# biod/sambamba

Measured on AMD Instinct MI355X. Metric: depth_base_Mreads_per_s, higher is better.
Workload: dtype u8/u32

## Files before the change

sambamba_amd/csrc/inflate.hip:

```cpp
#include <cstdlib>

#include "common.hpp"
#include "inflate2_core.hpp"
#include "lz77_copy.hpp"
#include "kernels.hpp"

namespace sbx {

namespace {

constexpr int kInfThreads = 64;
constexpr int kLaneLds = 356;
constexpr int kLitSymOff = 0;
constexpr int kLitSymBytes = 324;
constexpr int kRingOff = 324;
constexpr int kClLenOff = 32;
constexpr int kLenTabBytes = 64, kDistTabBytes = 128;
constexpr int kLensScratch = 320;
constexpr int kScratchStride = inf2::kScratchBytes;
constexpr int kGeneralLensOff = inf2::kScratchTabs;
static_assert(kGeneralLensOff + kLensScratch <= kScratchStride, "scratch layout");

enum : uint32_t {
    INF_OK = 0,
// ... 456 lines not shown
            if (ncl_left) {
                br.refill();
                cl_len[kClOrder[cl_i++]] = (uint8_t)br.take(3);
                --ncl_left;
            }
            br.service();
        }
        if (dyn) {
            int k = 0;
            for (int l = 1; l <= 7; ++l)
                for (int s2 = 0; s2 < 19; ++s2)
                    if (cl_len[s2] == l) cl_sym[k++] = (uint8_t)s2;
            for (int s2 = 0; s2 < 19; ++s2) {
                uint32_t l = cl_len[s2];
#pragma unroll
                for (int q = 1; q < 8; ++q) ccnt[q] += (l == (uint32_t)q) ? 1u : 0u;
            }
            int32_t left = 1;
            bool ok = true;
#pragma unroll
            for (int l = 1; l <= 7; ++l) { left = (left << 1) - (int32_t)ccnt[l]; if (left < 0) ok = false; }
            if (!ok) { err = INF_BAD_CODELENS; active = false; dyn = false; }
        }
        {
            int i = 0;
            uint32_t prev = 0;
            const int total = nlit + ndist;
            bool more = dyn;
            while (__any(more)) {
                if (more) {
                    br.refill();
                    uint32_t code = 0, first = 0, index = 0, sym = 0xFFFFFFFFu;
                    int used = 0;
#pragma unroll
                    for (int l = 1; l <= 7; ++l) {
                        code |= (uint32_t)(br.buf >> (l - 1)) & 1u;
                        uint32_t c = ccnt[l];
                        if (used == 0 && code < first + c) {
                            sym = cl_sym[index + (code - first)];
                            used = l;
                        }
                        index += c;
                        first = (first + c) << 1;
                        code <<= 1;
                    }
                    if (sym >= 19) { err = INF_BAD_CODELENS; more = false; }
                    else {
                        br.drop(used);
                        if (sym < 16) {
                            lens[i++] = (uint8_t)sym;
                            prev = sym;
                        } else {
                            uint32_t rep, val;
                            if (sym == 16) { val = prev; rep = 3 + br.take(2); if (i == 0) { err = INF_BAD_CODELENS; more = false; rep = 0; } }
                            else if (sym == 17) { val = 0; rep = 3 + br.take(3); }
                            else { val = 0; rep = 11 + br.take(7); }
                            if (i + (int)rep > total) { err = INF_BAD_CODELENS; more = false; }
                            else {
                                for (uint32_t k = 0; k < rep; ++k) lens[i++] = (uint8_t)val;
                                prev = val;
                            }
                        }
                        if (i >= total) more = false;
                    }
                }
                br.service();
            }
            if (dyn && err == INF_OK && lens[256] == 0) err = INF_BAD_CODELENS;
            if (err != INF_OK) active = false;
        }
        bool sym_loop = huff && active;
        bool lit_in_14 = true, dist_in_12 = true;
        if (sym_loop) {
            if (!build_code<true, 14>(lens, nlit, lds, DS, CL, &lit_in_14)) { err = INF_BAD_CODELENS; active = false; sym_loop = false; }
            else if (!build_code<false, 12>(lens + nlit, ndist, lds, DS, CD, &dist_in_12)) { err = INF_BAD_CODELENS; active = false; sym_loop = false; }
        }
        uint32_t short_lit = __builtin_amdgcn_readfirstlane(__all(!sym_loop || lit_in_14) ? 1u : 0u);
        uint32_t short_dist = __builtin_amdgcn_readfirstlane(__all(!sym_loop || dist_in_12) ? 1u : 0u);
        asm volatile("" : "+s"(short_lit), "+s"(short_dist));

        if (__any(sym_loop)) do {
            br.service();
            em.flush();
            uint32_t msym = 0;
            uint32_t bad = INF_OK;
            static_assert(kLitPerIter * 15 <= 32, "one refill must cover the literal/length slots of an iteration");
            if (sym_loop) br.refill();
#pragma unroll
            for (int r = 0; r < kLitPerIter; ++r) {
                if (sym_loop && msym == 0 && bad == INF_OK) {
                    const uint32_t v = __brev((uint32_t)br.buf) >> 17;
                    int len;
                    uint32_t delta;
                    decode_len<7>(CL, v, short_lit, &len, &delta);
                    const int lc = len > 15 ? 15 : len;
                    const uint32_t idx0 = (delta + (v >> (15 - lc))) & 0x1FFu;
                    const uint32_t idx = idx0 > 287u ? 287u : idx0;
                    const uint32_t bo = 9u * idx;
                    uint16_t packed;
                    __builtin_memcpy(&packed, lds + kLitSymOff + (bo >> 3), 2);
                    const uint32_t sym = ((uint32_t)packed >> (bo & 7u)) & 0x1FFu;
                    br.drop(lc);
                    const bool ok = len <= 15 && idx0 <= 287u && sym <= 285u;
                    if (ok && sym < 256u) em.literal(sym);
                    sym_loop = !(ok && sym == 256u);
                    msym = ok && sym > 256u ? sym : 0u;
                    bad = ok ? INF_OK : INF_BAD_SYMBOL;
                }
            }
            em.park_lits();
            const uint32_t opos_now = opos + em.n_lit;
            if (opos_now > osize && bad == INF_OK) { bad = INF_OUTPUT_OVERRUN; msym = 0; }
            if (msym != 0) {
                br.refill();
                const uint32_t lt = len_tab[msym - 257u];
                const uint32_t le = lt >> 9, lb = lt & 0x1FFu;
                const uint32_t mlen = lb + br.take((int)le);
                const uint32_t dv = __brev((uint32_t)br.buf) >> 17;
                int dl;
                uint32_t ddelta;
                decode_len<6>(CD, dv, short_dist, &dl, &ddelta);
                const int dc = dl > 15 ? 15 : dl;
                const uint32_t didx0 = (ddelta + (dv >> (15 - dc))) & 0x1FFu;
                const uint32_t dsym = DS.get(didx0 > 29u ? 29u : didx0);
                br.drop(dc);
                const uint32_t dt = dist_tab[dsym];
                const uint32_t de = dt >> 16, db = dt & 0xFFFFu;
                const uint32_t dist = db + br.take((int)de);
                const bool code_ok = dl <= 15 && didx0 < 30u && dsym <= 29u && dist <= opos_now;
                const bool fits = opos_now + mlen <= osize;
                if (code_ok && fits) { opos += mlen; em.match(mlen, dist); }
                bad = !code_ok ? (uint32_t)INF_BAD_DISTANCE : !fits ? (uint32_t)INF_OUTPUT_OVERRUN : bad;
            }
            if (bad != INF_OK) { err = bad; active = false; sym_loop = false; }
        } while (__any(sym_loop));
        if (active && last) active = false;
    }
    em.finish();
    if (err == INF_OK && opos + em.n_lit != osize) err = INF_SIZE_MISMATCH;
    if (err == INF_OK && br.consumed() > in_bits) err = INF_INPUT_OVERRUN;
    if (live) {
        status[b] = err;
        n_entries[b] = em.n_ent;
    }
    if (tok_bytes) {
        unsigned long long t = live ? (unsigned long long)em.n_lit + 4ull * em.n_ent : 0ull;
        for (int d = 32; d >= 1; d >>= 1) t += __shfl_xor(t, d, 64);
        if (threadIdx.x == 0) atomicAdd(tok_bytes + (blockIdx.x & 63u), t);
    }
}


constexpr int kInf2Threads = 64;
__global__ __launch_bounds__(kInf2Threads) __attribute__((amdgpu_waves_per_eu(4, 4))) void k_huffman_decode2(
    const uint8_t* __restrict__ comp, const uint64_t* __restrict__ comp_off, const uint32_t* __restrict__ comp_len,
    const uint32_t* __restrict__ isize, const uint64_t* __restrict__ out_off, uint32_t n_blocks, uint32_t block0,
    uint8_t* __restrict__ lit_stream, uint32_t* __restrict__ ent_stream, uint32_t* __restrict__ n_entries,
    uint8_t* __restrict__ scratch, uint32_t* __restrict__ status, unsigned long long* __restrict__ tok_bytes) {
    extern __shared__ __attribute__((aligned(16))) uint8_t smem[];
    const uint32_t lane = threadIdx.x;
    const uint32_t b_raw = blockIdx.x * kInf2Threads + lane;
    const bool live = b_raw < n_blocks;
    const uint32_t b = live ? b_raw : n_blocks - 1;
    uint16_t* const len_tab = (uint16_t*)(smem + inf2::kWaveLds);
    uint32_t* const dist_tab = (uint32_t*)(smem + inf2::kWaveLds + inf2::kLenTabBytes);
    if (lane < 32u) inf2::rfc_tables_entry(lane, &len_tab[lane], &dist_tab[lane]);
    __syncthreads();
    const uint64_t oo = out_off[b];
    inf2::LaneIo io;
    io.in = comp + comp_off[b];
    io.in_bits = comp_len[b] * 8u;
    io.osize = isize[b];
    io.lit = lit_stream + lit_off(oo, block0 + b);
    io.ent = ent_stream + ent_off(oo, block0 + b);
    io.scratch = scratch + (size_t)b * kScratchStride;
    io.live = live;
    inf2::Lane L;
    const inf2::LaneResult R = L.run(io, smem, lane, len_tab, dist_tab);
    if (live) {
        status[b] = R.status;
        n_entries[b] = R.n_ent;
    }
    if (tok_bytes) {
        unsigned long long t = live && R.status == 0u ? (unsigned long long)R.n_lit + 4ull * R.n_ent : 0ull;
        for (int d = 32; d >= 1; d >>= 1) t += __shfl_xor(t, d, 64);
        if (lane == 0) atomicAdd(tok_bytes + (blockIdx.x & 63u), t);
    }
}

__global__ __launch_bounds__(64) void k_translate_literals(
    uint8_t* __restrict__ lit_stream, const uint64_t* __restrict__ out_off, uint32_t n_blocks, uint32_t block0,
    const uint8_t* __restrict__ scratch, const uint32_t* __restrict__ status) {
    __shared__ __attribute__((aligned(16))) uint8_t tabs[inf2::kMaxSeg * 256];
    __shared__ uint32_t seg_start[inf2::kMaxSeg + 1];
    const uint32_t b = blockIdx.x, lane = threadIdx.x;
    if (status[b] != INF_OK) return;
    const uint8_t* sc = scratch + (size_t)b * kScratchStride;
    const uint32_t* info = (const uint32_t*)(sc + inf2::kScratchInfo);
    const uint32_t n_seg = info[0], n_lit = info[1];
    if (n_seg == 0u || n_lit == 0u) return;
    for (uint32_t s = 0; s < n_seg; ++s) ((uint32_t*)tabs)[64u * s + lane] = ((const uint32_t*)(sc + inf2::kScratchTabs))[64u * s + lane];
    if (lane <= n_seg) seg_start[lane] = lane < n_seg ? info[2 + lane] : n_lit;
    __syncthreads();
    uint8_t* lit = lit_stream + lit_off(out_off[b], block0 + b);
    const uint32_t n_grp = (n_lit + 15u) >> 4;
    for (uint32_t g = lane; g < n_grp; g += 64) {
        u32x4 v = *(const u32x4*)(lit + 16u * g);
        const uint32_t p0 = 16u * g;
        uint32_t s0 = 0;
        while (s0 + 1u < n_seg && seg_start[s0 + 1u] <= p0) ++s0;
        const uint32_t next = seg_start[s0 + 1u];
        uint32_t w[4] = {v.x, v.y, v.z, v.w};
        if (next >= p0 + 16u || s0 + 1u >= n_seg) {
            const uint8_t* t = tabs + 256u * s0;
#pragma unroll
            for (int k = 0; k < 4; ++k) {
                const uint32_t x = w[k];
                w[k] = (uint32_t)t[x & 0xFFu] | (uint32_t)t[(x >> 8) & 0xFFu] << 8 | (uint32_t)t[(x >> 16) & 0xFFu] << 16 | (uint32_t)t[x >> 24] << 24;
            }
        } else {
            for (uint32_t i = 0; i < 16; ++i) {
                const uint32_t p = p0 + i;
                uint32_t sg = s0;
                while (sg + 1u < n_seg && seg_start[sg + 1u] <= p) ++sg;
                const uint32_t x = (w[i >> 2] >> (8u * (i & 3u))) & 0xFFu;
                const uint32_t y = tabs[256u * sg + x];
                w[i >> 2] = (w[i >> 2] & ~(0xFFu << (8u * (i & 3u)))) | y << (8u * (i & 3u));
            }
        }
        *(u32x4*)(lit + 16u * g) = u32x4{w[0], w[1], w[2], w[3]};
    }
}

constexpr int kResThreads = 256;
constexpr uint32_t kHistDefault = 2048, kSpanDefault = 1536;

__device__ __forceinline__ uint32_t wave_incl_scan(uint32_t v, uint32_t lane) {
    (void)lane;
    v += (uint32_t)__builtin_amdgcn_update_dpp(0, (int)v, 0x111, 0xF, 0xF, true);
    v += (uint32_t)__builtin_amdgcn_update_dpp(0, (int)v, 0x112, 0xF, 0xF, true);
    v += (uint32_t)__builtin_amdgcn_update_dpp(0, (int)v, 0x114, 0xF, 0xF, true);
    v += (uint32_t)__builtin_amdgcn_update_dpp(0, (int)v, 0x118, 0xF, 0xF, true);
    v += (uint32_t)__builtin_amdgcn_update_dpp(0, (int)v, 0x142, 0xA, 0xF, false);
    v += (uint32_t)__builtin_amdgcn_update_dpp(0, (int)v, 0x143, 0xC, 0xF, false);
    return v;
}

using lz::Short16;

__device__ __forceinline__ void coop_copy(uint64_t m, const uint8_t* sbase, uint32_t s, uint8_t* buf, uint32_t d, uint32_t n, uint32_t lane) {
    while (m) {
        uint32_t S[4], D[4], N[4], wa[4], wb[4];
#pragma unroll
        for (int j = 0; j < 4; ++j) {
            N[j] = 0; S[j] = 0; D[j] = 0;
            if (m) {
                const int r = __builtin_ctzll(m);
                m &= m - 1;
                S[j] = __builtin_amdgcn_readlane(s, r);
                D[j] = __builtin_amdgcn_readlane(d, r);
                N[j] = __builtin_amdgcn_readlane(n, r);
            }
        }
        const uint32_t off = 8 * lane;
#pragma unroll
        for (int j = 0; j < 4; ++j) {
            if (off < N[j]) {
                const uint32_t a = off + 4 <= N[j] ? off : N[j] - 4, c = off + 8 <= N[j] ? off + 4 : N[j] - 4;
                wa[j] = ldu32(sbase + S[j] + a);
                wb[j] = ldu32(sbase + S[j] + c);
            }
        }
#pragma unroll
        for (int j = 0; j < 4; ++j) {
            if (off < N[j]) {
                const uint32_t a = off + 4 <= N[j] ? off : N[j] - 4, c = off + 8 <= N[j] ? off + 4 : N[j] - 4;
                stu32(buf + D[j] + a, wa[j]);
                stu32(buf + D[j] + c, wb[j]);
            }
        }
    }
}

__device__ __forceinline__ void wave_copy(uint8_t* d, const uint8_t* s, uint32_t N, uint32_t lane) {
    if (N >= 4) {
        for (uint32_t off = 4 * lane; off < N; off += 256) {
            const uint32_t o2 = off + 4 <= N ? off : N - 4;
            stu32(d + o2, ldu32(s + o2));
        }
    } else if (lane < N) {
        d[lane] = s[lane];
    }
}

template <uint32_t kHist, uint32_t kSpanMax, bool kOwn32, bool kExact, uint32_t kAblate = 0, bool kTail16 = true>
__device__ __forceinline__ void lz77_resolve_body(
    const uint8_t* __restrict__ lit_stream, const uint32_t* __restrict__ ent_stream, const uint32_t* __restrict__ n_entries,
    const uint64_t* __restrict__ out_off, const uint32_t* __restrict__ isize, uint32_t n_blocks, uint32_t block0,
    uint8_t* out, const uint32_t* __restrict__ status) {
    extern __shared__ __attribute__((aligned(16))) uint8_t smem[];
    const uint32_t lane = threadIdx.x & 63u, wv = threadIdx.x >> 6;
    const uint32_t b = blockIdx.x * (kResThreads / 64) + wv;
    if (kOwn32) {
        uint32_t* tab = (uint32_t*)(smem + (kResThreads / 64) * (kHist + 1024u + kSpanMax + 16u));
        if (threadIdx.x < 32u) {
            const uint32_t d = (threadIdx.x >> 2) + 1u, j = threadIdx.x & 3u;
            tab[threadIdx.x] = lz::period_selector(d, j);
        }
        __syncthreads();
    }
    if (b >= n_blocks) return;
    if (status[b] != INF_OK) return;
    constexpr uint32_t kCap = kHist + 1024u + kSpanMax, kWaveLds = kCap + 16u;
    uint8_t* buf = smem + wv * kWaveLds;
    const uint32_t* per_sel = (const uint32_t*)(smem + (kResThreads / 64) * kWaveLds);
    const uint64_t oo = out_off[b];
    const uint8_t* lit = lit_stream + lit_off(oo, block0 + b);
    const uint32_t* ent = ent_stream + ent_off(oo, block0 + b);
    uint8_t* o = out + oo;
    const uint32_t ne = n_entries[b];
    uint32_t opos = 0, lpos = 0;
    uint32_t base = 0;

    uint32_t e_next = lane < ne ? ent[lane] : 0u;
    for (uint32_t e0 = 0; e0 < ne;) {
        uint32_t e = e_next;
        const uint32_t in_batch = ne - e0 < 64u ? ne - e0 : 64u;
        uint32_t lr = e >> 24, len = e & 511u;
        const uint32_t dist = ((e >> 9) & 0x7FFFu) + 1u;
        uint32_t tot = lr + len;
        const uint32_t pk = wave_incl_scan(tot | (lr << 16), lane);
        const uint32_t take = __popcll(__ballot(lane < in_batch && (pk & 0xFFFFu) <= kSpanMax));
        if (lane >= take) { lr = 0; len = 0; tot = 0; }
        const uint32_t pk_last = __builtin_amdgcn_readlane(pk, take - 1);
        const uint32_t span = pk_last & 0xFFFFu, lspan = pk_last >> 16;
        e0 += take;
        e_next = (e0 + lane < ne) ? ent[e0 + lane] : 0u;
        if (!(kAblate & 32u) && opos - base + kSpanMax > kCap) {
            const uint32_t nb = (opos - kHist) & ~15u, delta = nb - base, keep = opos - nb;
            for (uint32_t i = 16 * lane; i < keep; i += 1024) {
// ... 238 lines not shown
```

sambamba_amd/csrc/inflate2_core.hpp:

```cpp
#pragma once
#include <cstdint>
#include <cstring>

#if defined(__HIPCC__)
#include <hip/hip_runtime.h>
#define SBX_HD __host__ __device__ __forceinline__
#else
#define SBX_HD inline
#endif

namespace sbx {
namespace inf2 {

constexpr uint32_t kNeedsGeneral = 100;
constexpr int kMaxSeg = 6;
constexpr int kScratchLens = 0;
constexpr int kScratchInfo = 160;
constexpr int kScratchTabs = 256;
constexpr int kScratchBytes = kScratchTabs + kMaxSeg * 256;

constexpr int kRingDw = 9;
constexpr int kOffRing = 0;
constexpr int kOffLitStage = kOffRing + 256 * kRingDw;
constexpr int kOffEntStage = kOffLitStage + 256 * 4;
constexpr int kOffAux = kOffEntStage + 256 * 8;
constexpr int kSymEntries = 30;
constexpr int kOffLenSym = kOffAux + 128 * 16;
constexpr int kOffDistSym = kOffLenSym + 64 * kSymEntries;
constexpr int kWaveLds = kOffDistSym + 64 * kSymEntries;
constexpr int kLenTabBytes = 64, kDistTabBytes = 128;

constexpr uint32_t kNone = 0xFFu, kStop = 0x1FFu;

#if defined(__HIP_DEVICE_COMPILE__)
typedef short s16x2 __attribute__((ext_vector_type(2)));
typedef unsigned short u16x2 __attribute__((ext_vector_type(2)));
SBX_HD uint32_t alignbit(uint32_t hi, uint32_t lo, uint32_t s) { return __builtin_amdgcn_alignbit(hi, lo, s); }
SBX_HD uint32_t brev32(uint32_t x) { return __builtin_bitreverse32(x); }
SBX_HD bool wave_any(bool x) { return __any(x) != 0; }
SBX_HD uint32_t bfe(uint32_t x, uint32_t off, uint32_t width) { return __builtin_amdgcn_ubfe(x, off, width); }
SBX_HD uint32_t pair_mask(uint32_t lim1, uint32_t vv) {
    const s16x2 d = __builtin_bit_cast(s16x2, lim1) - __builtin_bit_cast(s16x2, vv);
    return __builtin_bit_cast(uint32_t, __builtin_bit_cast(u16x2, d) >> 15);
}
SBX_HD uint32_t pair_dot(uint32_t m, uint32_t dd, uint32_t acc) {
    return __builtin_amdgcn_udot2(__builtin_bit_cast(u16x2, m), __builtin_bit_cast(u16x2, dd), acc, false);
}
#else
SBX_HD uint32_t alignbit(uint32_t hi, uint32_t lo, uint32_t s) { return (uint32_t)(((((uint64_t)hi) << 32) | lo) >> (s & 31u)); }
SBX_HD uint32_t brev32(uint32_t x) {
    x = ((x >> 1) & 0x55555555u) | ((x & 0x55555555u) << 1);
    x = ((x >> 2) & 0x33333333u) | ((x & 0x33333333u) << 2);
    x = ((x >> 4) & 0x0F0F0F0Fu) | ((x & 0x0F0F0F0Fu) << 4);
    x = ((x >> 8) & 0x00FF00FFu) | ((x & 0x00FF00FFu) << 8);
    return (x >> 16) | (x << 16);
}
SBX_HD bool wave_any(bool x) { return x; }
SBX_HD uint32_t bfe(uint32_t x, uint32_t off, uint32_t width) { return width == 0 ? 0u : (x >> (off & 31u)) & (width >= 32 ? 0xFFFFFFFFu : ((1u << width) - 1u)); }
SBX_HD uint32_t pair_mask(uint32_t lim1, uint32_t vv) {
    const uint32_t a = (uint16_t)((uint16_t)lim1 - (uint16_t)vv), b = (uint16_t)((uint16_t)(lim1 >> 16) - (uint16_t)(vv >> 16));
    return (a >> 15) | ((b >> 15) << 16);
}
SBX_HD uint32_t pair_dot(uint32_t m, uint32_t dd, uint32_t acc) { return acc + (m & 0xFFFFu) * (dd & 0xFFFFu) + (m >> 16) * (dd >> 16); }
#endif

SBX_HD uint32_t make_entry2(uint32_t lit_run, uint32_t len, uint32_t dist) { return (lit_run << 24) | ((dist - 1u) << 9) | len; }

struct u32x4h { uint32_t x, y, z, w; };


struct Code {
    uint32_t lim1[8], dd[8];
    uint32_t d1;
    uint32_t d1_lo;
};

#if defined(__HIP_DEVICE_COMPILE__)
SBX_HD uint32_t splat16(uint32_t v) { const u16x2 x = {(unsigned short)v, (unsigned short)v}; return __builtin_bit_cast(uint32_t, x); }
#define SBX_KEEP_BRANCH() asm volatile("")
#else
SBX_HD uint32_t splat16(uint32_t v) { return v | (v << 16); }
#define SBX_KEEP_BRANCH() (void)0
#endif

template <int kFrom, int kTo>
SBX_HD uint32_t decode_pairs(const Code& C, uint32_t v, uint32_t acc) {
    const uint32_t vv = splat16(v);
    uint32_t m[kTo - kFrom > 0 ? kTo - kFrom : 1];
#pragma unroll
    for (int j = kFrom; j < kTo; ++j) m[j - kFrom] = pair_mask(C.lim1[j], vv);
#pragma unroll
    for (int j = kFrom; j < kTo; ++j) acc = pair_dot(m[j - kFrom], C.dd[j], acc);
    return acc;
}

template <bool kPlain>
SBX_HD uint32_t decode_lit(const Code& C, uint32_t v) { return kPlain ? decode_pairs<1, 7>(C, v, C.d1_lo) : decode_pairs<0, 8>(C, v, C.d1); }
template <bool kPlain>
SBX_HD uint32_t decode_dist(const Code& C, uint32_t v) { return kPlain ? decode_pairs<1, 6>(C, v, C.d1_lo) : decode_pairs<0, 8>(C, v, C.d1); }

constexpr uint64_t kClOrderLo = 16ull | 17ull << 5 | 18ull << 10 | 0ull << 15 | 8ull << 20 | 7ull << 25 | 9ull << 30 | 6ull << 35 | 10ull << 40 | 5ull << 45 | 11ull << 50 | 4ull << 55;
constexpr uint64_t kClOrderHi = 12ull | 3ull << 5 | 13ull << 10 | 2ull << 15 | 14ull << 20 | 1ull << 25 | 15ull << 30;

struct LaneIo {
    const uint8_t* in;
    uint32_t in_bits;
    uint32_t osize;
    uint8_t* lit;
    uint32_t* ent;
    uint8_t* scratch;
    bool live;
};
struct LaneResult {
    uint32_t status;
    uint32_t n_ent, n_lit;
};

struct Lane {
    uint8_t* W;
    uint32_t l4, l2, l1;
    const uint16_t* len_tab;
    const uint32_t* dist_tab;
    const uint8_t* gp;
    u32x4h pend;
    uint32_t wr_dw;
    uint32_t bitpos;
    uint32_t hi, lo;
    uint32_t n_lit, n_ent, lit_mark, opos;
    uint32_t lit_flushed, ent_flushed;
    uint8_t* lit;
    uint32_t* ent;

    SBX_HD uint32_t& dw(int off, uint32_t j) const { return *(uint32_t*)(W + off + 256u * j + l4); }
    SBX_HD uint16_t& h16(int off, uint32_t e) const { return *(uint16_t*)(W + off + 128u * e + l2); }
    SBX_HD uint8_t& b8(int off, uint32_t e) const { return W[off + 64u * e + l1]; }

    SBX_HD static u32x4h load16(const uint8_t* p) {
        u32x4h v;
#if defined(__HIP_DEVICE_COMPILE__)
        typedef uint32_t u32x4g __attribute__((ext_vector_type(4)));
        const u32x4g q = *(const __attribute__((address_space(1))) u32x4g*)(uintptr_t)p;
        v.x = q.x; v.y = q.y; v.z = q.z; v.w = q.w;
#else
        __builtin_memcpy(&v, p, 16);
#endif
        return v;
    }
    SBX_HD static void store16(void* p, u32x4h v) { __builtin_memcpy(p, &v, 16); }

    SBX_HD void put_chunk(u32x4h v) {
        const uint32_t s = wr_dw & 7u;
        dw(kOffRing, s) = v.x; dw(kOffRing, s + 1) = v.y; dw(kOffRing, s + 2) = v.z; dw(kOffRing, s + 3) = v.w;
        if (s == 0u) dw(kOffRing, 8) = v.x;
        wr_dw += 4;
    }
    SBX_HD void init_input(const uint8_t* p) {
        const uint32_t lead = (uint32_t)((uintptr_t)p & 3u);
        const uint8_t* a = p - lead;
        wr_dw = 0;
        put_chunk(load16(a));
        put_chunk(load16(a + 16));
        pend = load16(a + 32);
        gp = a + 48;
        bitpos = 8u * lead;
    }
    SBX_HD void service() {
        if ((bitpos >> 5) + 4u >= wr_dw) {
            put_chunk(pend);
            pend = load16(gp);
            gp += 16;
        }
    }
    SBX_HD uint32_t window32(uint32_t at) const {
        const uint32_t t = (at >> 5) & 7u;
        return alignbit(dw(kOffRing, t + 1), dw(kOffRing, t), at);
    }
    SBX_HD uint64_t window64(uint32_t at) const {
        const uint32_t t = (at >> 5) & 7u;
        return ((((uint64_t)dw(kOffRing, t + 1)) << 32) | dw(kOffRing, t)) >> (at & 31u);
    }

    SBX_HD void push_lit(uint32_t rank) {
        lo = alignbit(hi, lo, 8);
        hi = alignbit(rank, hi, 8);
        ++n_lit;
    }
    SBX_HD void stage_lit_dword(uint32_t n_lit0) {
        if ((n_lit >> 2) != (n_lit0 >> 2)) {
            const uint32_t d = (n_lit & 3u) ? alignbit(hi, lo, 24) : hi;
            dw(kOffLitStage, ((n_lit >> 2) - 1u) & 3u) = d;
        }
    }
    SBX_HD void stage_entry(uint32_t e) {
        dw(kOffEntStage, n_ent & 7u) = e;
        ++n_ent;
    }
    SBX_HD u32x4h lit_group() const {
        u32x4h g;
        g.x = dw(kOffLitStage, 0); g.y = dw(kOffLitStage, 1); g.z = dw(kOffLitStage, 2); g.w = dw(kOffLitStage, 3);
        return g;
    }
    SBX_HD u32x4h ent_group(uint32_t grp) const {
        const uint32_t b = 4u * (grp & 1u);
        u32x4h g;
        g.x = dw(kOffEntStage, b); g.y = dw(kOffEntStage, b + 1u); g.z = dw(kOffEntStage, b + 2u); g.w = dw(kOffEntStage, b + 3u);
        return g;
    }
    SBX_HD void flush_groups() {
        if ((n_lit >> 4) != lit_flushed) {
            store16(lit + 16u * lit_flushed, lit_group());
            ++lit_flushed;
        }
        while ((n_ent >> 2) != ent_flushed) {
            store16(ent + 4u * ent_flushed, ent_group(ent_flushed));
            ++ent_flushed;
        }
    }
    SBX_HD void flush_one() {
        const bool rl = (n_lit >> 4) != lit_flushed, re = (n_ent >> 2) != ent_flushed;
        if (rl || re) {
            const uint32_t b = rl ? 0u : 4u * (ent_flushed & 1u);
            const int off = rl ? kOffLitStage : kOffEntStage;
            u32x4h g;
            g.x = dw(off, b); g.y = dw(off, b + 1u); g.z = dw(off, b + 2u); g.w = dw(off, b + 3u);
            uint8_t* const p = rl ? lit + 16u * lit_flushed : (uint8_t*)(ent + 4u * ent_flushed);
            store16(p, g);
            lit_flushed += rl ? 1u : 0u;
            ent_flushed += rl ? 0u : 1u;
        }
    }
    SBX_HD bool have_input() const { return (wr_dw << 5) - bitpos >= 96u; }

    template <bool kPlain>
    SBX_HD void symbol_loop(const Code& CL, const Code& CD, const LaneIo& io, bool huff, uint32_t& err, bool& active) {
    uint32_t st = huff ? kNone : kStop;
    if (wave_any(st != kStop)) do {
#pragma unroll
        for (int half = 0; half < 2; ++half) {
        if (half == 0) service(); else flush_one();
        const bool input = have_input();
        const uint32_t n_lit0 = n_lit;
        if (st == kNone && input) {
            const uint32_t w = window32(bitpos);
            const uint32_t v1 = brev32(w) >> 17;
            const uint32_t acc1 = decode_lit<kPlain>(CL, v1);
            const uint32_t len1 = (acc1 >> 13) + 1u;
            const uint32_t a1 = h16(kOffAux, len1);
            const uint32_t v2 = brev32(w >> len1) >> 17;
            const uint32_t acc2 = decode_lit<kPlain>(CL, v2);
            const uint32_t len2 = (acc2 >> 13) + 1u;
            const uint32_t a2 = h16(kOffAux, len2);
            const uint32_t idx1 = ((v1 >> (15u - len1)) + acc1) & 0x1FFu, idx2 = ((v2 >> (15u - len2)) + acc2) & 0x1FFu;
            const uint32_t litend1 = a1 & 0x1FFu, E1 = a1 >> 9, litend2 = a2 & 0x1FFu, E2 = a2 >> 9;
            const bool lit1 = idx1 < litend1, lit2 = lit1 && idx2 < litend2;
            {
                const uint32_t nlo = alignbit(hi, lo, 8), nhi = alignbit(idx1 - E1, hi, 8);
                lo = lit1 ? nlo : lo;
                hi = lit1 ? nhi : hi;
            }
            {
                const uint32_t nlo = alignbit(hi, lo, 8), nhi = alignbit(idx2 - E2, hi, 8);
                lo = lit2 ? nlo : lo;
                hi = lit2 ? nhi : hi;
            }
            n_lit += (lit1 ? 1u : 0u) + (lit2 ? 1u : 0u);
            bitpos += len1 + (lit1 ? len2 : 0u);
            const uint32_t j1 = (idx1 - litend1 + E1) & 31u, j2 = (idx2 - litend2 + E2) & 31u;
            st = !lit1 ? j1 : !lit2 ? j2 : kNone;
        }
        stage_lit_dword(n_lit0);
        const uint32_t opos_now = opos + n_lit;
        const uint32_t run_len = n_lit - lit_mark;
        const bool split = run_len >= 255u;
        const bool do_d = !split && st < 32u && input;
        bool eob = false, m_ok = false;
        uint32_t m_e = 0, m_bits = 0, m_len = 0;
        if (do_d) {
            const uint32_t s5 = b8(kOffLenSym, st < (uint32_t)kSymEntries ? st : 0u);
            const uint32_t lt = len_tab[(s5 - 1u) & 31u];
            uint64_t w64 = window64(bitpos);
            const uint32_t le = lt >> 9, lb = lt & 0x1FFu;
            const uint32_t mlen = lb + bfe((uint32_t)w64, 0, le);
            w64 >>= le;
            const uint32_t dv = brev32((uint32_t)w64) >> 17;
            const uint32_t acc = decode_dist<kPlain>(CD, dv);
            const uint32_t dm1 = acc >> 13;
            const uint32_t dl = dm1 + 1u;
            const uint32_t didx = ((dv >> ((14u - (dm1 & 15u)) & 31u)) + acc) & 0x1FFu;
            const uint32_t dsym = b8(kOffDistSym, didx < (uint32_t)kSymEntries ? didx : 0u);
            const uint32_t dt = dist_tab[dsym & 31u];
            w64 >>= dl;
            const uint32_t de = dt >> 16, db = dt & 0xFFFFu;
            const uint32_t dist = db + bfe((uint32_t)w64, 0, de);
            eob = s5 == 0u && st < (uint32_t)kSymEntries;
            m_ok = st < (uint32_t)kSymEntries && s5 - 1u < 29u && dm1 <= 14u && didx < (uint32_t)kSymEntries && dist <= opos_now && opos_now + mlen <= io.osize;
            m_e = make_entry2(run_len, mlen, dist);
            m_bits = le + dl + de;
            m_len = mlen;
        }
        const bool bad = (do_d && !eob && !m_ok) || (st != kStop && opos_now > io.osize);
        if (split || m_ok) stage_entry(split ? make_entry2(255, 0, 1) : m_e);
        lit_mark = split ? lit_mark + 255u : m_ok ? n_lit : lit_mark;
        bitpos += m_ok ? m_bits : 0u;
        opos += m_ok ? m_len : 0u;
        st = do_d ? (eob ? kStop : kNone) : st;
        if (bad) { err = 1; st = kStop; active = false; }
        }
    } while (wave_any(st != kStop));
    }

    SBX_HD LaneResult run(const LaneIo& io, uint8_t* W_, uint32_t lane, const uint16_t* len_tab_, const uint32_t* dist_tab_) {
        W = W_;
        l4 = 4u * lane; l2 = 2u * lane; l1 = lane;
        len_tab = len_tab_;
        dist_tab = dist_tab_;
        lit = io.lit;
        ent = io.ent;
        hi = lo = 0;
        n_lit = n_ent = lit_mark = opos = lit_flushed = ent_flushed = 0;
        init_input(io.in);
        const uint32_t lead_bits = bitpos;
        uint32_t* const lens32 = (uint32_t*)(io.scratch + kScratchLens);
        uint32_t* const info = (uint32_t*)(io.scratch + kScratchInfo);
        uint32_t n_seg = 0;
        uint32_t err = 0;
        Code CL, CD;
#pragma unroll
        for (int j = 0; j < 8; ++j) { CL.lim1[j] = CL.dd[j] = CD.lim1[j] = CD.dd[j] = 0; }
        CL.d1 = CL.d1_lo = CD.d1 = CD.d1_lo = 0;

        bool active = io.live && !(io.osize == 0 && io.in_bits == 0);
        bool last = false;
        while (wave_any(active)) {
            service();
            uint32_t btype = 3;
            if (active) {
                const uint32_t w = window32(bitpos);
                last = (w & 1u) != 0;
                btype = (w >> 1) & 3u;
                bitpos += 3;
                if (btype == 0u || btype == 3u) { err = 1; active = false; }
                if (bitpos - lead_bits > io.in_bits) { err = 1; active = false; }
                if (n_seg >= (uint32_t)kMaxSeg) { err = 1; active = false; }
            }
            uint32_t nlit = 0, ndist = 0;
            bool has_eob = false;
            if (active) {
#pragma unroll
                for (uint32_t l = 0; l < 16; ++l) { h16(kOffAux, l) = 0; b8(kOffLenSym, l) = 0; }
            }
            if (active && btype == 1u) {
                for (uint32_t i = 0; i < 40; ++i)
                    lens32[i] = i < 18 ? 0x88888888u : i < 32 ? 0x99999999u : i < 35 ? 0x77777777u : i < 36 ? 0x88888888u : i < 39 ? 0x55555555u : 0x00555555u;
                nlit = 288; ndist = 30;
                h16(kOffAux, 7) = (uint16_t)(24u << 9);
                h16(kOffAux, 8) = (uint16_t)(144u | 8u << 9);
                h16(kOffAux, 9) = (uint16_t)112u;
                b8(kOffLenSym, 5) = 30;
                has_eob = true;
            }
            bool dyn = active && btype == 2u;
            uint64_t clen = 0;
            int ncl_left = 0;
            if (dyn) {
                const uint32_t w = window32(bitpos);
                nlit = (w & 31u) + 257u;
                ndist = ((w >> 5) & 31u) + 1u;
                ncl_left = (int)((w >> 10) & 15u) + 4;
                bitpos += 14;
                if (nlit > 286u || ndist > 30u) { err = 1; active = false; dyn = false; ncl_left = 0; }
            }
            for (uint32_t i = 0; wave_any(ncl_left != 0); ++i) {
                service();
                if (ncl_left != 0) {
                    const uint32_t ord = (uint32_t)((i < 12u ? kClOrderLo >> (5u * i) : kClOrderHi >> (5u * (i - 12u))) & 31u);
                    const uint32_t w = window32(bitpos);
                    clen |= (uint64_t)(w & 7u) << (3u * ord);
                    bitpos += 3;
                    --ncl_left;
                }
            }
            uint64_t ccnt = 0;
            uint64_t csa = 0, csb = 0;
            if (dyn) {
                for (uint32_t s = 0; s < 19; ++s) ccnt += 1ull << (5u * (uint32_t)((clen >> (3u * s)) & 7u));
                uint32_t k = 0;
                for (uint32_t l = 1; l <= 7; ++l)
                    for (uint32_t s = 0; s < 19; ++s)
                        if (((clen >> (3u * s)) & 7u) == l) {
                            if (k < 12u) csa |= (uint64_t)s << (5u * k); else csb |= (uint64_t)s << (5u * (k - 12u));
                            ++k;
                        }
                int32_t left = 1;
                bool ok = true;
                for (uint32_t l = 1; l <= 7; ++l) { left = (left << 1) - (int32_t)((ccnt >> (5u * l)) & 31u); if (left < 0) ok = false; }
                if (!ok) { err = 1; active = false; dyn = false; }
            }
            {
                uint32_t i = 0, prev = 0, nib = 0;
                const uint32_t total = nlit + ndist;
                bool more = dyn;
                while (wave_any(more)) {
                    service();
                    if (more) {
                        const uint32_t w = window32(bitpos);
                        uint32_t code = 0, first = 0, index = 0, sym = 99, used = 0;
#pragma unroll
                        for (uint32_t l = 1; l <= 7; ++l) {
                            code |= (w >> (l - 1)) & 1u;
                            const uint32_t c = (uint32_t)(ccnt >> (5u * l)) & 31u;
                            if (used == 0u && code < first + c) {
                                const uint32_t q = index + (code - first);
                                sym = (uint32_t)((q < 12u ? csa >> (5u * q) : csb >> (5u * (q - 12u))) & 31u);
                                used = l;
                            }
                            index += c;
                            first = (first + c) << 1;
                            code <<= 1;
                        }
                        uint32_t rep = 0, val = 0;
                        if (used == 0u || sym >= 19u) { err = 1; more = false; }
                        else {
                            const uint32_t x = w >> used;
                            if (sym < 16u) { rep = 1; val = sym; prev = sym; bitpos += used; }
                            else if (sym == 16u) { rep = 3u + (x & 3u); val = prev; bitpos += used + 2u; if (i == 0u) { err = 1; more = false; rep = 0; } }
                            else if (sym == 17u) { rep = 3u + (x & 7u); val = 0; prev = 0; bitpos += used + 3u; }
                            else { rep = 11u + (x & 127u); val = 0; prev = 0; bitpos += used + 7u; }
                            if (i + rep > total) { err = 1; more = false; rep = 0; }
                        }
                        while (rep != 0u) {
                            if (val != 0u) {
                                if (i < 256u) h16(kOffAux, val) += 1u;
                                else if (i < nlit) { h16(kOffAux, val) += 512u; if (i == 256u) has_eob = true; }
                                else b8(kOffLenSym, val) += 1u;
                            }
                            nib |= val << (4u * (i & 7u));
                            ++i;
                            if ((i & 7u) == 0u) { lens32[(i >> 3) - 1u] = nib; nib = 0; }
                            --rep;
                        }
                        if (more && i >= total) {
                            more = false;
                            if (i & 7u) lens32[i >> 3] = nib;
                        }
                    }
                }
                if (dyn && err == 0u && !has_eob) err = 1;
                if (err != 0u) { active = false; dyn = false; }
            }
            bool huff = active;
            bool dist_in12 = true, dist_no12 = true, lit_in14 = true, lit_no12 = true;
            if (huff) {
                uint32_t first = 0, offs = 0, lim_prev = 0, D_prev = 0, lim_a = 0, dd_a = 0;
                int32_t left = 1;
                bool ok = true;
#pragma unroll
                for (uint32_t l = 1; l <= 16; ++l) {
                    uint32_t lim, D;
                    if (l <= 15) {
                        const uint32_t c = b8(kOffLenSym, l);
                        left = (left << 1) - (int32_t)c;
                        if (left < 0) ok = false;
                        lim = (first + c) << (15u - l);
                        D = offs - first;
                        b8(kOffLenSym, l) = (uint8_t)offs;
                        offs += c;
                        first = (first + c) << 1;
                        if (l == 2) dist_no12 = offs == 0u;
                        if (l == 12) dist_in12 = lim == 32768u;
                    } else { lim = 32768u; D = D_prev; }
                    if (l == 1) CD.d1 = D & 0x1FFu;
                    else {
                        const uint32_t ddh = ((D - D_prev) & 0x1FFu) | 0x2000u;
                        const uint32_t lm = l - 1;
                        if (lm & 1u) { lim_a = (lim_prev - 1u) & 0xFFFFu; dd_a = ddh; }
                        else { CD.lim1[(lm >> 1) - 1u] = lim_a | ((lim_prev - 1u) & 0xFFFFu) << 16; CD.dd[(lm >> 1) - 1u] = dd_a | ddh << 16; }
                    }
                    lim_prev = lim; D_prev = D;
                }
                CD.lim1[7] = lim_a | 32767u << 16;
                CD.dd[7] = dd_a | 0x2000u << 16;
                CD.d1_lo = CD.d1 + (CD.dd[0] & 0xFFFFu) + (CD.dd[0] >> 16);
                if (!ok) { err = 1; active = false; huff = false; }
            }
            if (huff) {
                for (uint32_t base = nlit & ~7u; wave_any(huff && base < nlit + ndist); base += 8) {
                    if (huff && base < nlit + ndist) {
                        const uint32_t w = lens32[base >> 3];
#pragma unroll
                        for (uint32_t n = 0; n < 8; ++n) {
                            const uint32_t s = base + n, l = (w >> (4u * n)) & 15u;
                            if (s >= nlit && s < nlit + ndist && l != 0u) {
                                const uint32_t idx = b8(kOffLenSym, l);
                                b8(kOffLenSym, l) = (uint8_t)(idx + 1u);
                                if (idx < (uint32_t)kSymEntries) b8(kOffDistSym, idx) = (uint8_t)(s - nlit);
                            }
                        }
                    }
                }
            }
            if (huff) {
                uint32_t first = 0, offs = 0, lim_prev = 0, D_prev = 0, lim_a = 0, dd_a = 0, litbase = 0, E = 0;
                int32_t left = 1;
                bool ok = true;
#pragma unroll
                for (uint32_t l = 1; l <= 16; ++l) {
                    uint32_t lim, D;
                    if (l <= 15) {
                        const uint32_t cc = h16(kOffAux, l);
                        const uint32_t c_lit = cc & 0x1FFu, c_non = cc >> 9, c = c_lit + c_non;
                        left = (left << 1) - (int32_t)c;
                        if (left < 0) ok = false;
                        lim = (first + c) << (15u - l);
                        D = offs - first;
                        h16(kOffAux, l) = (uint16_t)(litbase | E << 9);
                        litbase += c_lit;
                        E += c_non;
                        offs += c;
                        first = (first + c) << 1;
                        if (l == 2) lit_no12 = offs == 0u;
                        if (l == 14) lit_in14 = lim == 32768u;
                    } else { lim = 32768u; D = D_prev; }
                    if (l == 1) CL.d1 = D & 0x1FFu;
                    else {
                        const uint32_t ddh = ((D - D_prev) & 0x1FFu) | 0x2000u;
                        const uint32_t lm = l - 1;
                        if (lm & 1u) { lim_a = (lim_prev - 1u) & 0xFFFFu; dd_a = ddh; }
                        else { CL.lim1[(lm >> 1) - 1u] = lim_a | ((lim_prev - 1u) & 0xFFFFu) << 16; CL.dd[(lm >> 1) - 1u] = dd_a | ddh << 16; }
                    }
                    lim_prev = lim; D_prev = D;
                }
                CL.lim1[7] = lim_a | 32767u << 16;
                CL.dd[7] = dd_a | 0x2000u << 16;
                CL.d1_lo = CL.d1 + (CL.dd[0] & 0xFFFFu) + (CL.dd[0] >> 16);
                if (!ok || left != 0) { err = 1; active = false; huff = false; }
            }
            uint8_t* const tab = io.scratch + kScratchTabs + 256u * (n_seg < (uint32_t)kMaxSeg ? n_seg : 0u);
            if (huff) {
                for (uint32_t base = 0; wave_any(huff && base < nlit); base += 8) {
                    if (huff && base < nlit) {
                        const uint32_t w = lens32[base >> 3];
#pragma unroll
                        for (uint32_t n = 0; n < 8; ++n) {
                            const uint32_t s = base + n, l = (w >> (4u * n)) & 15u;
                            if (s < nlit && l != 0u) {
                                const uint32_t p = h16(kOffAux, l);
                                if (s < 256u) { h16(kOffAux, l) = (uint16_t)(p + 1u); tab[p & 0xFFu] = (uint8_t)s; }
                                else { h16(kOffAux, l) = (uint16_t)(p + 512u); if ((p >> 9) < (uint32_t)kSymEntries) b8(kOffLenSym, p >> 9) = (uint8_t)(s - 256u); }
                            }
                        }
                    }
                }
                uint32_t fin = h16(kOffAux, 15);
#pragma unroll
                for (uint32_t l = 15; l >= 1; --l) {
                    const uint32_t below = l > 1 ? (uint32_t)h16(kOffAux, l - 1) : 0u;
                    const uint32_t E_l = below >> 9;
                    h16(kOffAux, l) = (uint16_t)(((fin & 0x1FFu) + E_l) | E_l << 9);
                    fin = below;
                }
                info[2 + n_seg] = n_lit;
                ++n_seg;
            }
            bool plain = lit_no12 && lit_in14 && dist_no12 && dist_in12;
#if defined(__HIP_DEVICE_COMPILE__)
            plain = __builtin_amdgcn_readfirstlane(__all(!huff || plain) ? 1u : 0u) != 0u;
#endif
            if (plain) symbol_loop<true>(CL, CD, io, huff, err, active);
            else symbol_loop<false>(CL, CD, io, huff, err, active);
            if (active && bitpos - lead_bits > io.in_bits) { err = 1; active = false; }
            if (active && last) active = false;
        }
        flush_groups();
        {
            uint32_t run_len = n_lit - lit_mark;
            while (wave_any(run_len != 0u)) {
                if (run_len != 0u) {
                    const uint32_t r = run_len > 255u ? 255u : run_len;
                    stage_entry(make_entry2(r, 0, 1));
                    run_len -= r;
                }
                flush_groups();
            }
        }
        if (n_lit & 3u) dw(kOffLitStage, (n_lit >> 2) & 3u) = hi >> (8u * (4u - (n_lit & 3u)));
        if (n_lit & 15u) store16(lit + 16u * (n_lit >> 4), lit_group());
        if (n_ent & 3u) store16(ent + 4u * (n_ent >> 2), ent_group(n_ent >> 2));
        if (err == 0u && opos + n_lit != io.osize) err = 1;
        if (err == 0u && bitpos - lead_bits > io.in_bits) err = 1;
        if (io.live) {
            info[0] = err == 0u ? n_seg : 0u;
            info[1] = n_lit;
        }
        LaneResult R;
        R.status = err == 0u ? 0u : kNeedsGeneral;
        R.n_ent = n_ent;
        R.n_lit = n_lit;
        return R;
    }
};

SBX_HD void rfc_tables_entry(uint32_t i, uint16_t* len_e, uint32_t* dist_e) {
    const uint32_t t = i - 4u;
    const bool direct = i < 8u || i >= 28u;
    const uint32_t le = direct ? 0u : t >> 2;
    const uint32_t lb = i < 8u ? i + 3u : i >= 28u ? 258u : ((4u + (t & 3u)) << le) + 3u;
    *len_e = (uint16_t)(lb | le << 9);
    const uint32_t de = i < 4u ? 0u : ((i >> 1) - 1u) & 15u;
    const uint32_t db = i < 4u ? i + 1u : ((2u + (i & 1u)) << de) + 1u;
    *dist_e = db | de << 16;
}

}
}
```

Before: 1024.

## Make inflate symbol loop branchless and use sign-bit pair masks in plain decode

Makes the per-lane Huffman symbol loop branch-free. Literal and match decode now run every iteration with predicated results, literal pushes use one variable-width alignbit, flush and entry staging are unconditional, and the match validity check is folded into a single sign test. In the plain path the pair mask keeps the raw sign bits, so it skips a shift, and d1_lo is pre-shifted to match. An ablation template parameter is threaded through, and the default of 0 keeps full behaviour. The aim is to cut divergence and instruction count in the wave-wide loop, at the cost of always doing the full decode work even on lanes that are idle.

```diff
diff --git a/sambamba_amd/csrc/inflate.hip b/sambamba_amd/csrc/inflate.hip
--- a/sambamba_amd/csrc/inflate.hip
+++ b/sambamba_amd/csrc/inflate.hip
@@ -632,11 +632,14 @@
 
 
 constexpr int kInf2Threads = 64;
-__global__ __launch_bounds__(kInf2Threads) __attribute__((amdgpu_waves_per_eu(4, 4))) void k_huffman_decode2(
-    const uint8_t* __restrict__ comp, const uint64_t* __restrict__ comp_off, const uint32_t* __restrict__ comp_len,
-    const uint32_t* __restrict__ isize, const uint64_t* __restrict__ out_off, uint32_t n_blocks, uint32_t block0,
-    uint8_t* __restrict__ lit_stream, uint32_t* __restrict__ ent_stream, uint32_t* __restrict__ n_entries,
-    uint8_t* __restrict__ scratch, uint32_t* __restrict__ status, unsigned long long* __restrict__ tok_bytes) {
+#define SBX_K1A_ARGS                                                                                                                   \
+    const uint8_t* __restrict__ comp, const uint64_t* __restrict__ comp_off, const uint32_t* __restrict__ comp_len,                  \
+        const uint32_t* __restrict__ isize, const uint64_t* __restrict__ out_off, uint32_t n_blocks, uint32_t block0,                 \
+        uint8_t* __restrict__ lit_stream, uint32_t* __restrict__ ent_stream, uint32_t* __restrict__ n_entries,                        \
+        uint8_t* __restrict__ scratch, uint32_t* __restrict__ status, unsigned long long* __restrict__ tok_bytes
+#define SBX_K1A_PASS comp, comp_off, comp_len, isize, out_off, n_blocks, block0, lit_stream, ent_stream, n_entries, scratch, status, tok_bytes
+template <uint32_t kAblate>
+__device__ __forceinline__ void huffman_decode2_body(SBX_K1A_ARGS) {
     extern __shared__ __attribute__((aligned(16))) uint8_t smem[];
     const uint32_t lane = threadIdx.x;
     const uint32_t b_raw = blockIdx.x * kInf2Threads + lane;
@@ -656,7 +659,7 @@
     io.scratch = scratch + (size_t)b * kScratchStride;
     io.live = live;
     inf2::Lane L;
-    const inf2::LaneResult R = L.run(io, smem, lane, len_tab, dist_tab);
+    const inf2::LaneResult R = L.run<kAblate>(io, smem, lane, len_tab, dist_tab);
     if (live) {
         status[b] = R.status;
         n_entries[b] = R.n_ent;
@@ -666,6 +669,9 @@
         for (int d = 32; d >= 1; d >>= 1) t += __shfl_xor(t, d, 64);
         if (lane == 0) atomicAdd(tok_bytes + (blockIdx.x & 63u), t);
     }
+}
+__global__ __launch_bounds__(kInf2Threads) __attribute__((amdgpu_waves_per_eu(4, 4))) void k_huffman_decode2(SBX_K1A_ARGS) {
+    huffman_decode2_body<0>(SBX_K1A_PASS);
 }
 
 __global__ __launch_bounds__(64) void k_translate_literals(
diff --git a/sambamba_amd/csrc/inflate2_core.hpp b/sambamba_amd/csrc/inflate2_core.hpp
--- a/sambamba_amd/csrc/inflate2_core.hpp
+++ b/sambamba_amd/csrc/inflate2_core.hpp
@@ -43,6 +43,9 @@
     const s16x2 d = __builtin_bit_cast(s16x2, lim1) - __builtin_bit_cast(s16x2, vv);
     return __builtin_bit_cast(uint32_t, __builtin_bit_cast(u16x2, d) >> 15);
 }
+SBX_HD uint32_t pair_sign(uint32_t lim1, uint32_t vv) {
+    return __builtin_bit_cast(uint32_t, __builtin_bit_cast(s16x2, lim1) - __builtin_bit_cast(s16x2, vv)) & 0x80008000u;
+}
 SBX_HD uint32_t pair_dot(uint32_t m, uint32_t dd, uint32_t acc) {
     return __builtin_amdgcn_udot2(__builtin_bit_cast(u16x2, m), __builtin_bit_cast(u16x2, dd), acc, false);
 }
@@ -61,6 +64,7 @@
     const uint32_t a = (uint16_t)((uint16_t)lim1 - (uint16_t)vv), b = (uint16_t)((uint16_t)(lim1 >> 16) - (uint16_t)(vv >> 16));
     return (a >> 15) | ((b >> 15) << 16);
 }
+SBX_HD uint32_t pair_sign(uint32_t lim1, uint32_t vv) { return (pair_mask(lim1, vv) << 15) & 0x80008000u; }
 SBX_HD uint32_t pair_dot(uint32_t m, uint32_t dd, uint32_t acc) { return acc + (m & 0xFFFFu) * (dd & 0xFFFFu) + (m >> 16) * (dd >> 16); }
 #endif
 
@@ -83,21 +87,23 @@
 #define SBX_KEEP_BRANCH() (void)0
 #endif
 
-template <int kFrom, int kTo>
+template <int kFrom, int kTo, bool kSign = false>
 SBX_HD uint32_t decode_pairs(const Code& C, uint32_t v, uint32_t acc) {
     const uint32_t vv = splat16(v);
     uint32_t m[kTo - kFrom > 0 ? kTo - kFrom : 1];
 #pragma unroll
-    for (int j = kFrom; j < kTo; ++j) m[j - kFrom] = pair_mask(C.lim1[j], vv);
+    for (int j = kFrom; j < kTo; ++j) m[j - kFrom] = kSign ? pair_sign(C.lim1[j], vv) : pair_mask(C.lim1[j], vv);
 #pragma unroll
     for (int j = kFrom; j < kTo; ++j) acc = pair_dot(m[j - kFrom], C.dd[j], acc);
     return acc;
 }
 
 template <bool kPlain>
-SBX_HD uint32_t decode_lit(const Code& C, uint32_t v) { return kPlain ? decode_pairs<1, 7>(C, v, C.d1_lo) : decode_pairs<0, 8>(C, v, C.d1); }
+SBX_HD uint32_t decode_lit(const Code& C, uint32_t v) { return kPlain ? decode_pairs<1, 7, true>(C, v, C.d1_lo) : decode_pairs<0, 8>(C, v, C.d1); }
 template <bool kPlain>
-SBX_HD uint32_t decode_dist(const Code& C, uint32_t v) { return kPlain ? decode_pairs<1, 6>(C, v, C.d1_lo) : decode_pairs<0, 8>(C, v, C.d1); }
+SBX_HD uint32_t decode_dist(const Code& C, uint32_t v) { return kPlain ? decode_pairs<1, 6, true>(C, v, C.d1_lo) : decode_pairs<0, 8>(C, v, C.d1); }
+template <bool kPlain> constexpr uint32_t acc_idx_shift() { return kPlain ? 15u : 0u; }
+template <bool kPlain> constexpr uint32_t acc_len_shift() { return kPlain ? 28u : 13u; }
 
 constexpr uint64_t kClOrderLo = 16ull | 17ull << 5 | 18ull << 10 | 0ull << 15 | 8ull << 20 | 7ull << 25 | 9ull << 30 | 6ull << 35 | 10ull << 40 | 5ull << 45 | 11ull << 50 | 4ull << 55;
 constexpr uint64_t kClOrderHi = 12ull | 3ull << 5 | 13ull << 10 | 2ull << 15 | 14ull << 20 | 1ull << 25 | 15ull << 30;
@@ -180,16 +186,10 @@
         return ((((uint64_t)dw(kOffRing, t + 1)) << 32) | dw(kOffRing, t)) >> (at & 31u);
     }
 
-    SBX_HD void push_lit(uint32_t rank) {
-        lo = alignbit(hi, lo, 8);
-        hi = alignbit(rank, hi, 8);
-        ++n_lit;
-    }
-    SBX_HD void stage_lit_dword(uint32_t n_lit0) {
-        if ((n_lit >> 2) != (n_lit0 >> 2)) {
-            const uint32_t d = (n_lit & 3u) ? alignbit(hi, lo, 24) : hi;
-            dw(kOffLitStage, ((n_lit >> 2) - 1u) & 3u) = d;
-        }
+    SBX_HD void stage_lit_dword() {
+        const uint32_t r = n_lit & 3u;
+        const uint32_t d = r ? alignbit(hi, lo, 32u - 8u * r) : hi;
+        dw(kOffLitStage, ((n_lit >> 2) - 1u) & 3u) = d;
     }
     SBX_HD void stage_entry(uint32_t e) {
         dw(kOffEntStage, n_ent & 7u) = e;
@@ -218,97 +218,95 @@
     }
     SBX_HD void flush_one() {
         const bool rl = (n_lit >> 4) != lit_flushed, re = (n_ent >> 2) != ent_flushed;
-        if (rl || re) {
-            const uint32_t b = rl ? 0u : 4u * (ent_flushed & 1u);
-            const int off = rl ? kOffLitStage : kOffEntStage;
-            u32x4h g;
-            g.x = dw(off, b); g.y = dw(off, b + 1u); g.z = dw(off, b + 2u); g.w = dw(off, b + 3u);
-            uint8_t* const p = rl ? lit + 16u * lit_flushed : (uint8_t*)(ent + 4u * ent_flushed);
-            store16(p, g);
-            lit_flushed += rl ? 1u : 0u;
-            ent_flushed += rl ? 0u : 1u;
-        }
+        const uint32_t b = rl ? 0u : 4u * (ent_flushed & 1u);
+        const int off = rl ? kOffLitStage : kOffEntStage;
+        u32x4h g;
+        g.x = dw(off, b); g.y = dw(off, b + 1u); g.z = dw(off, b + 2u); g.w = dw(off, b + 3u);
+        uint8_t* const p = rl ? lit + 16u * lit_flushed : (uint8_t*)(ent + 4u * ent_flushed);
+        if (rl || re) store16(p, g);
+        lit_flushed += rl ? 1u : 0u;
+        ent_flushed += !rl && re ? 1u : 0u;
     }
     SBX_HD bool have_input() const { return (wr_dw << 5) - bitpos >= 96u; }
 
-    template <bool kPlain>
+    template <bool kPlain, uint32_t kAblate = 0>
     SBX_HD void symbol_loop(const Code& CL, const Code& CD, const LaneIo& io, bool huff, uint32_t& err, bool& active) {
     uint32_t st = huff ? kNone : kStop;
     if (wave_any(st != kStop)) do {
 #pragma unroll
         for (int half = 0; half < 2; ++half) {
-        if (half == 0) service(); else flush_one();
+        if (half == 0) service();
+        else if (kAblate & 2u) { lit_flushed = n_lit >> 4; ent_flushed = n_ent >> 2; }
+        else flush_one();
         const bool input = have_input();
-        const uint32_t n_lit0 = n_lit;
-        if (st == kNone && input) {
-            const uint32_t w = window32(bitpos);
-            const uint32_t v1 = brev32(w) >> 17;
-            const uint32_t acc1 = decode_lit<kPlain>(CL, v1);
-            const uint32_t len1 = (acc1 >> 13) + 1u;
-            const uint32_t a1 = h16(kOffAux, len1);
-            const uint32_t v2 = brev32(w >> len1) >> 17;
-            const uint32_t acc2 = decode_lit<kPlain>(CL, v2);
-            const uint32_t len2 = (acc2 >> 13) + 1u;
-            const uint32_t a2 = h16(kOffAux, len2);
-            const uint32_t idx1 = ((v1 >> (15u - len1)) + acc1) & 0x1FFu, idx2 = ((v2 >> (15u - len2)) + acc2) & 0x1FFu;
-            const uint32_t litend1 = a1 & 0x1FFu, E1 = a1 >> 9, litend2 = a2 & 0x1FFu, E2 = a2 >> 9;
-            const bool lit1 = idx1 < litend1, lit2 = lit1 && idx2 < litend2;
-            {
-                const uint32_t nlo = alignbit(hi, lo, 8), nhi = alignbit(idx1 - E1, hi, 8);
-                lo = lit1 ? nlo : lo;
-                hi = lit1 ? nhi : hi;
-            }
-            {
-                const uint32_t nlo = alignbit(hi, lo, 8), nhi = alignbit(idx2 - E2, hi, 8);
-                lo = lit2 ? nlo : lo;
-                hi = lit2 ? nhi : hi;
-            }
-            n_lit += (lit1 ? 1u : 0u) + (lit2 ? 1u : 0u);
-            bitpos += len1 + (lit1 ? len2 : 0u);
-            const uint32_t j1 = (idx1 - litend1 + E1) & 31u, j2 = (idx2 - litend2 + E2) & 31u;
-            st = !lit1 ? j1 : !lit2 ? j2 : kNone;
-        }
-        stage_lit_dword(n_lit0);
+        const bool go = st == kNone && input;
+        const uint32_t w = window32(bitpos);
+        const uint32_t v1 = brev32(w) >> 17;
+        const uint32_t acc1 = decode_lit<kPlain>(CL, v1);
+        const uint32_t len1 = (acc1 >> acc_len_shift<kPlain>()) + 1u;
+        const uint32_t a1 = h16(kOffAux, len1);
+        const uint32_t v2 = brev32(w >> len1) >> 17;
+        const uint32_t acc2 = decode_lit<kPlain>(CL, v2);
+        const uint32_t len2 = (acc2 >> acc_len_shift<kPlain>()) + 1u;
+        const uint32_t a2 = h16(kOffAux, len2);
+        const uint32_t idx1 = ((v1 >> ((15u - len1) & 31u)) + (acc1 >> acc_idx_shift<kPlain>())) & 0x1FFu;
+        const uint32_t idx2 = ((v2 >> ((15u - len2) & 31u)) + (acc2 >> acc_idx_shift<kPlain>())) & 0x1FFu;
+        const uint32_t litend1 = a1 & 0x1FFu, E1 = a1 >> 9, litend2 = a2 & 0x1FFu, E2 = a2 >> 9;
+        const bool lit1 = go && idx1 < litend1, lit2 = lit1 && idx2 < litend2;
+        const uint32_t k = (lit1 ? 1u : 0u) + (lit2 ? 1u : 0u);
+        if (!(kAblate & 1u)) {
+            const uint32_t r12 = (idx1 - E1) + ((idx2 - E2) << 8);
+            lo = alignbit(hi, lo, 8u * k);
+            hi = alignbit(r12, hi, 8u * k);
+        }
+        n_lit += k;
+        bitpos += go ? len1 + (lit1 ? len2 : 0u) : 0u;
+        const uint32_t j1 = (idx1 - litend1 + E1) & 31u, j2 = (idx2 - litend2 + E2) & 31u;
+        st = !go ? st : !lit1 ? j1 : !lit2 ? j2 : kNone;
+        if (!(kAblate & 1u)) stage_lit_dword();
         const uint32_t opos_now = opos + n_lit;
         const uint32_t run_len = n_lit - lit_mark;
         const bool split = run_len >= 255u;
         const bool do_d = !split && st < 32u && input;
-        bool eob = false, m_ok = false;
-        uint32_t m_e = 0, m_bits = 0, m_len = 0;
-        if (do_d) {
-            const uint32_t s5 = b8(kOffLenSym, st < (uint32_t)kSymEntries ? st : 0u);
-            const uint32_t lt = len_tab[(s5 - 1u) & 31u];
-            uint64_t w64 = window64(bitpos);
-            const uint32_t le = lt >> 9, lb = lt & 0x1FFu;
-            const uint32_t mlen = lb + bfe((uint32_t)w64, 0, le);
-            w64 >>= le;
-            const uint32_t dv = brev32((uint32_t)w64) >> 17;
-            const uint32_t acc = decode_dist<kPlain>(CD, dv);
-            const uint32_t dm1 = acc >> 13;
-            const uint32_t dl = dm1 + 1u;
-            const uint32_t didx = ((dv >> ((14u - (dm1 & 15u)) & 31u)) + acc) & 0x1FFu;
-            const uint32_t dsym = b8(kOffDistSym, didx < (uint32_t)kSymEntries ? didx : 0u);
-            const uint32_t dt = dist_tab[dsym & 31u];
-            w64 >>= dl;
-            const uint32_t de = dt >> 16, db = dt & 0xFFFFu;
-            const uint32_t dist = db + bfe((uint32_t)w64, 0, de);
-            eob = s5 == 0u && st < (uint32_t)kSymEntries;
-            m_ok = st < (uint32_t)kSymEntries && s5 - 1u < 29u && dm1 <= 14u && didx < (uint32_t)kSymEntries && dist <= opos_now && opos_now + mlen <= io.osize;
-            m_e = make_entry2(run_len, mlen, dist);
-            m_bits = le + dl + de;
-            m_len = mlen;
+        const uint32_t s5 = b8(kOffLenSym, st < (uint32_t)kSymEntries ? st : 0u);
+        const uint32_t lt = len_tab[(s5 - 1u) & 31u];
+        uint64_t w64 = window64(bitpos);
+        const uint32_t le = lt >> 9, lb = lt & 0x1FFu;
+        const uint32_t mlen = lb + bfe((uint32_t)w64, 0, le);
+        w64 >>= le;
+        const uint32_t dv = brev32((uint32_t)w64) >> 17;
+        const uint32_t acc = decode_dist<kPlain>(CD, dv);
+        const uint32_t dm1 = acc >> acc_len_shift<kPlain>();
+        const uint32_t dl = dm1 + 1u;
+        const uint32_t didx = ((dv >> ((14u - dm1) & 31u)) + (acc >> acc_idx_shift<kPlain>())) & 0x1FFu;
+        const uint32_t dsym = b8(kOffDistSym, didx < (uint32_t)kSymEntries ? didx : 0u);
+        const uint32_t dt = dist_tab[dsym & 31u];
+        w64 >>= dl;
+        const uint32_t de = dt >> 16, db = dt & 0xFFFFu;
+        const uint32_t dist = db + bfe((uint32_t)w64, 0, de);
+        const bool sym_ok = st < (uint32_t)kSymEntries;
+        const bool eob = do_d && s5 == 0u && sym_ok;
+        bool m_ok;
+        if (kAblate & 4u) {
+            m_ok = do_d && sym_ok && s5 != 0u;
+        } else {
+            uint32_t neg = ((uint32_t)kSymEntries - 1u - st) | (s5 - 1u) | (29u - s5) | (opos_now - dist) | (io.osize - opos_now - mlen);
+            if (!kPlain) neg |= (14u - dm1) | ((uint32_t)kSymEntries - 1u - didx);
+            m_ok = do_d && (int32_t)neg >= 0;
         }
         const bool bad = (do_d && !eob && !m_ok) || (st != kStop && opos_now > io.osize);
-        if (split || m_ok) stage_entry(split ? make_entry2(255, 0, 1) : m_e);
+        if (!(kAblate & 2u)) dw(kOffEntStage, n_ent & 7u) = split ? make_entry2(255, 0, 1) : make_entry2(run_len, mlen, dist);
+        n_ent += split || m_ok ? 1u : 0u;
         lit_mark = split ? lit_mark + 255u : m_ok ? n_lit : lit_mark;
-        bitpos += m_ok ? m_bits : 0u;
-        opos += m_ok ? m_len : 0u;
+        bitpos += m_ok ? le + dl + de : 0u;
+        opos += m_ok ? mlen : 0u;
         st = do_d ? (eob ? kStop : kNone) : st;
         if (bad) { err = 1; st = kStop; active = false; }
         }
     } while (wave_any(st != kStop));
     }
 
+    template <uint32_t kAblate = 0>
     SBX_HD LaneResult run(const LaneIo& io, uint8_t* W_, uint32_t lane, const uint16_t* len_tab_, const uint32_t* dist_tab_) {
         W = W_;
         l4 = 4u * lane; l2 = 2u * lane; l1 = lane;
@@ -480,7 +478,7 @@
                 }
                 CD.lim1[7] = lim_a | 32767u << 16;
                 CD.dd[7] = dd_a | 0x2000u << 16;
-                CD.d1_lo = CD.d1 + (CD.dd[0] & 0xFFFFu) + (CD.dd[0] >> 16);
+                CD.d1_lo = (CD.d1 + (CD.dd[0] & 0xFFFFu) + (CD.dd[0] >> 16)) << 15;
                 if (!ok) { err = 1; active = false; huff = false; }
             }
             if (huff) {
@@ -532,7 +530,7 @@
                 }
                 CL.lim1[7] = lim_a | 32767u << 16;
                 CL.dd[7] = dd_a | 0x2000u << 16;
-                CL.d1_lo = CL.d1 + (CL.dd[0] & 0xFFFFu) + (CL.dd[0] >> 16);
+                CL.d1_lo = (CL.d1 + (CL.dd[0] & 0xFFFFu) + (CL.dd[0] >> 16)) << 15;
                 if (!ok || left != 0) { err = 1; active = false; huff = false; }
             }
             uint8_t* const tab = io.scratch + kScratchTabs + 256u * (n_seg < (uint32_t)kMaxSeg ? n_seg : 0u);
@@ -566,8 +564,8 @@
 #if defined(__HIP_DEVICE_COMPILE__)
             plain = __builtin_amdgcn_readfirstlane(__all(!huff || plain) ? 1u : 0u) != 0u;
 #endif
-            if (plain) symbol_loop<true>(CL, CD, io, huff, err, active);
-            else symbol_loop<false>(CL, CD, io, huff, err, active);
+            if (plain) symbol_loop<true, kAblate>(CL, CD, io, huff, err, active);
+            else symbol_loop<false, kAblate>(CL, CD, io, huff, err, active);
             if (active && bitpos - lead_bits > io.in_bits) { err = 1; active = false; }
             if (active && last) active = false;
         }
```

Result: faster. 1035 (median of 6 runs) (+1.1%).
